# benjaminrwilson/range-view-3d-detection

Measured on AMD Instinct MI355X. Metric: sweeps/sec (fwd+bwd, 64x2048x5 range image), higher is better.
Workload: dtype bf16

## Files before the change

include/rv3d.h:

```cpp
#ifndef RV3D_H_
#define RV3D_H_

#include <stdint.h>

#ifdef __cplusplus
extern "C" {
#endif

typedef void* rvStream;

int rv_version(void);
const char* rv_last_error(void);

typedef struct {
    int32_t kh, kw;
    int32_t stride_w;
    int32_t pad_h, pad_w;
    int32_t cu, cv;
} rvTapGeom;

int32_t rv_pad_channels(int32_t c);

int64_t rv_packed_weight_bytes(const rvTapGeom* g);

int rv_pack_weight(const rvTapGeom* g, const float* T, void* gather_w, void* scatter_w, rvStream stream);

int64_t rv_pack_batch_entry_bytes(void);
int rv_pack_batch_fill(const rvTapGeom* g, const float* T, void* gather_w, void* scatter_w, void* host_entries);
int rv_pack_batch(const void* dev_table, int32_t n_entries, rvStream stream);

int rv_fold_geom(const rvTapGeom* g, rvTapGeom* folded);
int rv_pack_weight_folded(const rvTapGeom* g, const float* T, void* gather_w_folded, rvStream stream);
int rv_pack_batch_fill_folded(const rvTapGeom* g, const float* T, void* gather_w_folded, void* host_entry);
int rv_unfold_weight_grad(const rvTapGeom* g, const float* dT_folded, float* dT, int32_t accumulate, rvStream stream);

int rv_unpack_weight_grad(const rvTapGeom* g, const float* packed, float* dT, int32_t accumulate, rvStream stream);

#define RV_IN_AFFINE 1
#define RV_IN_RELU 2
#define RV_OUT_F32 4
#define RV_OUT_BIAS 8
#define RV_OUT_STATS 16
#define RV_OUT_ACCUM 32
#define RV_OUT_RELU 64
#define RV_OUT_RES_RELU 256
#define RV_WGRAD_TORCH_LAYOUT 128
#define RV_SEL_SMALL_GRIDS (1 << 20)
#define RV_SEL_SMALL_GRIDS6 (1 << 21)
#define RV_SEL_NO_GEN6 (1 << 22)
#define RV_SEL_NO_GEN5 (1 << 23)
#define RV_SEL_NO_POINTWISE (1 << 24)
#define RV_SEL_NO_POINTWISE_BWD (1 << 25)
#define RV_SEL_MASK (63 << 20)

typedef struct {
    int32_t N, H, Wu, Wv;
    int32_t ld_src, ld_dst;
    int32_t flags;
} rvTapShape;

int32_t rv_tap_stats_rows(const rvTapGeom* g, const rvTapShape* s, int32_t scatter);
int rv_tap_launch_info(const rvTapGeom* g, const rvTapShape* s, int32_t scatter, int32_t* host_info);
#define RV_STATS_SCRATCH_ROWS 128

int rv_tap_gather(const rvTapGeom* g, const rvTapShape* s, const void* V, const float* in_scale,
                  const float* in_shift, const void* gather_w, const float* bias, void* U,
                  float* stats_partial, rvStream stream);

int rv_tap_scatter(const rvTapGeom* g, const rvTapShape* s, const void* U, const float* in_scale,
                   const float* in_shift, const void* scatter_w, const float* bias, void* V,
                   float* stats_partial, rvStream stream);

int rv_tap_residual(const rvTapGeom* g, const rvTapShape* s, int32_t scatter, const void* src, const void* w, const float* bias,
                    const void* res, int32_t ld_res, void* dst, rvStream stream);

typedef struct rvBnbEpilogue {
    const void* y;
    int32_t ld_y;
    int32_t flags;
    const float* scale;
    const float* shift;
    const float* mean;
    const float* invstd;
    float* partial;
} rvBnbEpilogue;
int32_t rv_tap_bnb_rows(const rvTapGeom* g, const rvTapShape* s, int32_t scatter);
int rv_tap_data_grad_bnb(const rvTapGeom* g, const rvTapShape* s, int32_t scatter, const void* dout, const void* w, void* dx,
                         const rvBnbEpilogue* e, rvStream stream);

int64_t rv_tap_wgrad_workspace_bytes(const rvTapGeom* g, const rvTapShape* s);
int rv_tap_wgrad_info(const rvTapGeom* g, const rvTapShape* s, int32_t* host_info);
int rv_tap_wgrad(const rvTapGeom* g, const rvTapShape* s, const void* U, int32_t ld_u, const void* V, int32_t ld_v,
                 const float* in_scale, const float* in_shift, int32_t v_affine, float* dT_packed,
                 void* workspace, rvStream stream);

int rv_reduce_rows(const float* partial, int32_t rows, int32_t cols, float* out, rvStream stream);
int rv_reduce_rows_count(const float* partial, int32_t rows, int32_t cols, float count, float* out, float* out_copy, rvStream stream);
int rv_bn_finalize(const float* partial, int32_t rows, int32_t c, int64_t count, const float* gamma,
                   const float* beta, float eps, float momentum, float* running_mean, float* running_var,
                   float* scale, float* shift, float* mean, float* invstd, rvStream stream);
int rv_bn_fold_eval(int32_t c, const float* gamma, const float* beta, const float* running_mean,
                    const float* running_var, float eps, float* scale, float* shift, rvStream stream);

#define RV_EW_RELU_A 1
#define RV_EW_RELU_B 2
#define RV_EW_RELU_OUT 4
int rv_ew_combine(int64_t pixels, int32_t c, const void* a, int32_t ld_a, const float* a_scale,
                  const float* a_shift, const void* b, int32_t ld_b, const float* b_scale,
                  const float* b_shift, void* out, int32_t ld_out, int32_t flags, rvStream stream);

#define RV_BNB_RELU_Z 1
#define RV_BNB_RES_ACCUM 2
#define RV_BNB_Y_FROM_INPUT 4
int32_t rv_bn_bwd_rows(int64_t pixels);
int rv_bn_bwd_reduce(int64_t pixels, int32_t c, const void* dout, int32_t ld_dout, const void* out, int32_t ld_out,
                     const void* y, int32_t ld_y, const float* scale, const float* shift, const float* mean,
                     const float* invstd, int32_t flags, float* partial, rvStream stream);
int rv_bn_bwd_reduce_pair(int64_t pixels, int32_t c, const void* dout, int32_t ld_dout, const void* out, int32_t ld_out,
                          const void* ya, int32_t ld_ya, const float* mean_a, const float* invstd_a, const void* yb, int32_t ld_yb,
                          const float* mean_b, const float* invstd_b, float* partial_a, float* partial_b, rvStream stream);
int rv_bn_bwd_apply_pair(int64_t pixels, int32_t c, const void* dout, int32_t ld_dout, const void* out, int32_t ld_out,
                         const void* ya, int32_t ld_ya, const float* mean_a, const float* invstd_a, const float* coef_a, void* dya,
                         int32_t ld_dya, const void* yb, int32_t ld_yb, const float* mean_b, const float* invstd_b,
                         const float* coef_b, void* dyb, int32_t ld_dyb, rvStream stream);
int rv_bn_bwd_finalize(const float* partial, int32_t rows, int32_t c, int64_t count, const float* gamma,
                       const float* invstd, float* dgamma, float* dbeta, int32_t accumulate, float* coef,
                       rvStream stream);
int rv_bn_bwd_apply(int64_t pixels, int32_t c, const void* dout, int32_t ld_dout, const void* out, int32_t ld_out,
                    const void* y, int32_t ld_y, const float* scale, const float* shift, const float* mean,
                    const float* invstd, const float* coef, int32_t flags, void* dy, int32_t ld_dy, void* dres,
                    int32_t ld_dres, rvStream stream);
int32_t rv_head_final_bwd_rows(int64_t pixels);
int rv_head_final_bwd_sums(int64_t pixels, int32_t c, const void* y, int32_t ld_y, const void* dY, int32_t ld_dy, const void* w_scatter,
                           const float* scale, const float* shift, const float* mean, const float* invstd, int32_t relu, float* partial,
                           float* dw_partial, rvStream stream);
int rv_head_final_bwd_apply(int64_t pixels, int32_t c, const void* y, int32_t ld_y, const void* dY, int32_t ld_dy, const void* w_scatter,
                            const float* scale, const float* shift, const float* mean, const float* invstd, int32_t relu, const float* coef,
                            void* dy, int32_t ld_out, rvStream stream);
int64_t rv_bn_bwd_smallk_workspace_bytes(int64_t pixels, int32_t c, int32_t cin);
int rv_bn_bwd_smallk(int64_t pixels, int32_t c, const void* dout, int32_t ld_dout, const void* out, int32_t ld_out,
                     const void* y, int32_t ld_y, const float* scale, const float* shift, const float* mean,
                     const float* invstd, int32_t flags, const void* v, int32_t ld_v, int32_t cin, const void* w_packed,
                     int32_t ld_w, const float* gamma, const float* stat_mean, const float* stat_invstd, int64_t count,
                     float* dgamma, float* dbeta, float* dW, void* workspace, rvStream stream);
int rv_bn_bwd_smallk_sums(int64_t pixels, int32_t c, const void* dout, int32_t ld_dout, const void* out, int32_t ld_out,
                          const void* y, int32_t ld_y, const float* scale, const float* shift, const float* mean,
                          const float* invstd, int32_t flags, const void* v, int32_t ld_v, int32_t cin, const void* w_packed,
                          int32_t ld_w, double* sums, double* moms, void* workspace, rvStream stream);
int rv_bn_bwd_smallk_from_sums(int32_t c, int32_t cin, const double* sums, const double* moms, const double* global_s01,
                               const void* w_packed, int32_t ld_w, const float* gamma, const float* stat_mean,
                               const float* stat_invstd, int64_t count, float* dgamma, float* dbeta, float* dW,
                               rvStream stream);
int64_t rv_smallk_forward_workspace_bytes(int32_t cin);
int rv_smallk_moments(const void* v, int32_t ld_v, int64_t pixels, int32_t cin, double* moments, void* workspace,
                      rvStream stream);
int rv_smallk_forward(const void* v, int32_t ld_v, int64_t pixels, int32_t cin, const void* w_packed, int32_t ld_w,
                      int32_t c, const double* moments, int64_t count, const float* gamma, const float* beta, float eps,
                      float momentum, float* running_mean, float* running_var, float* scale, float* shift, float* mean,
                      float* invstd, int32_t relu, void* h, int32_t ld_h, rvStream stream);
int rv_ew_mask_grad(int64_t pixels, int32_t c, const void* dout, int32_t ld_dout, const void* out, int32_t ld_out,
                    void* d, int32_t ld_d, int32_t accumulate, rvStream stream);

int rv_range_partition(const float* features_nchw, const float* cart_nchw, const uint8_t* mask, int32_t N, int32_t C, int32_t H, int32_t W,
                       const float* lower, const float* upper, int32_t bands, void* dst, int32_t ld_dst, rvStream stream);

int rv_nchw_f32_to_nhwc_bf16(const float* src, int32_t N, int32_t C, int32_t H, int32_t W, void* dst, int32_t ld_dst,
                             int32_t c_offset, rvStream stream);
int rv_nhwc_bf16_to_nchw_f32(const void* src, int32_t ld_src, int32_t c_offset, int32_t N, int32_t C, int32_t H,
                             int32_t W, float* dst, rvStream stream);
int rv_nhwc_f32_to_nchw_f32(const float* src, int32_t ld_src, int32_t N, int32_t C, int32_t H, int32_t W, float* dst,
                            rvStream stream);
int rv_nchw_f32_to_nhwc_f32(const float* src, int32_t N, int32_t C, int32_t H, int32_t W, float* dst, int32_t ld_dst,
                            rvStream stream);

int rv_meta_relative(const float* cart_nchw, int32_t N, int32_t H, int32_t W, void* rel, rvStream stream);
int rv_meta_modulate(const void* pos_raw, const float* scale, const float* shift, const void* feat, int32_t ld_feat,
                     int32_t N, int32_t H, int32_t W, int32_t C, void* geo, rvStream stream);
int rv_meta_modulate_bwd(const void* dgeo, const void* pos_raw, const float* scale, const float* shift,
                         const void* feat, int32_t ld_feat, int32_t N, int32_t H, int32_t W, int32_t C,
                         void* dpos_act, void* dfeat, int32_t ld_dfeat, rvStream stream);
int32_t rv_meta_bwd_rows(int32_t N, int32_t H, int32_t W);
int rv_meta_modulate_bwd_sums(const void* dgeo, const void* pos_raw, const float* scale, const float* shift,
                              const float* mean, const float* invstd, const void* feat, int32_t ld_feat, int32_t N,
                              int32_t H, int32_t W, int32_t C, void* dfeat, int32_t ld_dfeat, float* partial,
                              rvStream stream);
int rv_meta_modulate_bwd_apply(const void* dgeo, const void* pos_raw, const float* scale, const float* shift,
                               const float* mean, const float* invstd, const float* coef, const void* feat,
                               int32_t ld_feat, int32_t N, int32_t H, int32_t W, int32_t C, void* dy, rvStream stream);

int32_t rv_pos_forward_rows(int64_t pixels);
int rv_pos_forward(const void* rel, int32_t ld_rel, int32_t cin, int64_t pixels, const void* w1_packed, int32_t ld_w1,
                   const float* scale1, const float* shift1, const void* w2_packed, int32_t c, void* h1, void* y2,
                   float* stats_partial, rvStream stream);

int rv_pos_modulate_forward(const void* rel, int32_t ld_rel, int32_t cin, const void* w1_packed, int32_t ld_w1, const float* scale1,
                            const float* shift1, const void* w2_packed, int32_t c, const float* scale2, const float* shift2,
                            const void* feat, int32_t ld_feat, int32_t N, int32_t H, int32_t W, void* geo, rvStream stream);

int rv_pos_backward_sums(int64_t pixels, int32_t c, const void* dy2, const void* w2_scatter, const void* rel, int32_t ld_rel,
                         int32_t cin, const void* w1_packed, int32_t ld_w1, const float* scale1, const float* shift1,
                         const float* mean1, const float* invstd1, double* sums, double* moms, void* workspace, rvStream stream);

int32_t rv_optim_chunk_elems(void);
int rv_adamw_step(const void* tensors, const void* chunks, int32_t n_chunks, float* partial, double lr, double beta1,
                  double beta2, double eps, double weight_decay, int64_t step, double max_norm, float* total_norm,
                  rvStream stream);
// ... 185 lines not shown
```

range_view_3d_detection_amd/_lib.py:

```python

from __future__ import annotations

import ctypes
import os
import re
from typing import Dict, List, Optional

import torch

_HERE = os.path.dirname(os.path.abspath(__file__))
LIB_PATH = os.environ.get("RV3D_LIB") or os.path.join(_HERE, "librv3d_hip.so")
LIB_PATH_F16 = os.environ.get("RV3D_LIB_F16") or os.path.join(_HERE, "librv3d_hip_f16.so")
HEADER_PATH = os.path.join(os.path.dirname(_HERE), "include", "rv3d.h")

IN_AFFINE, IN_RELU, OUT_F32, OUT_BIAS, OUT_STATS, OUT_ACCUM, OUT_RELU = 1, 2, 4, 8, 16, 32, 64
OUT_RES_RELU = 256
WGRAD_TORCH_LAYOUT = 128
SEL_SMALL_GRIDS, SEL_SMALL_GRIDS6, SEL_NO_GEN6, SEL_NO_GEN5, SEL_NO_POINTWISE, SEL_NO_POINTWISE_BWD = 1 << 20, 1 << 21, 1 << 22, 1 << 23, 1 << 24, 1 << 25
SELECT = 0
EW_RELU_A, EW_RELU_B, EW_RELU_OUT = 1, 2, 4
BNB_RELU_Z, BNB_RES_ACCUM, BNB_Y_FROM_INPUT = 1, 2, 4
STATS_SCRATCH_ROWS = 128


class TapGeom(ctypes.Structure):
    _fields_ = [(n, ctypes.c_int32) for n in ("kh", "kw", "stride_w", "pad_h", "pad_w", "cu", "cv")]


class TapShape(ctypes.Structure):
    _fields_ = [(n, ctypes.c_int32) for n in ("N", "H", "Wu", "Wv", "ld_src", "ld_dst", "flags")]

    def __init__(self, *args, **kw) -> None:
        super().__init__(*args, **kw)
        self.flags |= SELECT


class select:

    def __init__(self, flags: int) -> None:
        self.flags = flags

    def __enter__(self):
        global SELECT
        self.old, SELECT = SELECT, SELECT | self.flags
        return self

    def __exit__(self, *exc):
        global SELECT
        SELECT = self.old


class BnbEpilogue(ctypes.Structure):

    _fields_ = [("y", ctypes.c_void_p), ("ld_y", ctypes.c_int32), ("flags", ctypes.c_int32), ("scale", ctypes.c_void_p), ("shift", ctypes.c_void_p),
                ("mean", ctypes.c_void_p), ("invstd", ctypes.c_void_p), ("partial", ctypes.c_void_p)]


class TargetLevel(ctypes.Structure):

    _fields_ = [("stride", ctypes.c_int32), ("use_range", ctypes.c_int32), ("lower", ctypes.c_double), ("upper", ctypes.c_double)]


class TargetOut(ctypes.Structure):

    _fields_ = [(n, ctypes.c_void_p) for n in ("labels", "panoptics", "reg_targets", "points_per_obj")]


class LossEntry(ctypes.Structure):

    _fields_ = [(n, ctypes.c_void_p) for n in ("logits", "regressands", "cart", "mask", "labels", "panoptics", "reg_targets", "points_per_obj",
                                               "num_objects", "soft_targets", "foreground", "d_logits", "d_regressands")] + \
               [(n, ctypes.c_int32) for n in ("ld_logits", "ld_reg", "B", "n_cls", "H", "W")]


class LossParams(ctypes.Structure):

    _fields_ = [("coding_weights", ctypes.c_float * 8)] + [(n, ctypes.c_float) for n in ("cls_weight", "reg_weight", "smoothing", "sigma", "alpha", "gamma")] + \
               [("azimuth_invariant", ctypes.c_int32)]


ML_MAX_LEVELS, ML_MAX_ENTRIES = 8, 16
AFFINITY_GAUSSIAN, AFFINITY_BEV = 0, 1
EVAL_MAX_THRESHOLDS, EVAL_MAX_DTS = 8, 1024
WAYMO_MAX_DTS, WAYMO_MAX_GTS, WAYMO_MAX_SWEEPS = 1024, 1024, 65536
WAYMO_NUM_CUTOFFS, WAYMO_NUM_BREAKDOWN_ROWS, WAYMO_NUM_RESULT_ROWS = 101, 16, 32


def loss_sums_len() -> int:
    return int(load().rv_detection_loss_sums_len())


class RvError(RuntimeError):
    pass


_lib: Optional[ctypes.CDLL] = None
_lib_f16: Optional[ctypes.CDLL] = None
_OPERAND = "bf16"


class operand:

    def __init__(self, tag: str) -> None:
        if tag not in ("bf16", "f16"):
            raise RvError(f"unknown operand type {tag!r}")
        self.tag = tag

    def __enter__(self):
        global _OPERAND
        self.old, _OPERAND = _OPERAND, self.tag
        return self

    def __exit__(self, *exc):
        global _OPERAND
        _OPERAND = self.old


def operand_tag() -> str:
    return _OPERAND


def act_dtype() -> "torch.dtype":
    return torch.float16 if _OPERAND == "f16" else torch.bfloat16


def declared_symbols() -> List[str]:
    text = open(HEADER_PATH).read()
    text = re.sub(r"/\*.*?\*/", "", text, flags=re.S)
    return sorted(set(re.findall(r"\b(rv_[a-z0-9_]+)\s*\(", text)))


def load(tag: Optional[str] = None) -> ctypes.CDLL:
    global _lib, _lib_f16
    tag = tag or _OPERAND
    if tag == "f16":
        if _lib_f16 is None:
            _lib_f16 = _dlopen(LIB_PATH_F16)
        return _lib_f16
    if _lib is None:
        _lib = _dlopen(LIB_PATH)
    return _lib


def _dlopen(path: str) -> ctypes.CDLL:
    if not os.path.exists(path):
        raise RvError(
            f"{path} is missing: build it with `python -c 'import __graft_entry__ as g; g.build()'` "
            "(hipcc --offload-arch=gfx950).  There is no CPU fallback."
        )
    if torch.cuda.device_count() > 0 and torch.cuda.is_available():
        torch.cuda.init()
    lib = ctypes.CDLL(path)
    lib.rv_last_error.restype = ctypes.c_char_p
    for name in ("rv_packed_weight_bytes", "rv_decode_num_candidates", "rv_wnms_workspace_bytes", "rv_tap_wgrad_workspace_bytes", "rv_bn_bwd_smallk_workspace_bytes", "rv_smallk_forward_workspace_bytes", "rv_nms_sweeps_workspace_bytes", "rv_nms_rotated_workspace_bytes", "rv_pack_batch_entry_bytes", "rv_soft_assign_workspace_bytes", "rv_db_paste_workspace_bytes",
                 "rv_eval_summarize_workspace_bytes", "rv_waymo_match_workspace_bytes"):
        if hasattr(lib, name):
            getattr(lib, name).restype = ctypes.c_int64
    return lib


def _as_arg(v):
    if v is None:
        return ctypes.c_void_p(0)
    if isinstance(v, (ctypes.Structure,)):
        return ctypes.byref(v)
    if isinstance(v, float):
        return ctypes.c_float(v)
    if isinstance(v, int):
        return ctypes.c_int64(v) if abs(v) > 0x7FFFFFFF else ctypes.c_int32(v)
    return v

# ... 75 lines not shown
```

range_view_3d_detection_amd/csrc/tapconv.h:

```cpp
#pragma once
#include "common.h"

constexpr int kMaxTaps = 24;
constexpr int kMaxPhases = 4;
constexpr int RV_OUT_BNB = 1 << 16;

struct TapTable {
    int32_t ntaps[kMaxPhases];
    int32_t w_first[kMaxPhases];
    int32_t dw_min[kMaxPhases], dw_max[kMaxPhases];
    int32_t w_tile[kMaxPhases];
    int32_t dh_min, rows;
    int8_t dh[kMaxPhases][kMaxTaps];
    int8_t dw[kMaxPhases][kMaxTaps];
    int8_t ky[kMaxPhases][kMaxTaps];
    int8_t kx[kMaxPhases][kMaxTaps];
};

struct TapConvArgs {
    const bf16_t* src;
    void* dst;
    const bf16_t* w;
    const float* in_scale;
    const float* in_shift;
    const float* bias;
    float* stats;
    int32_t N, H, W_src, W_dst;
    int32_t C_src, C_dst;
    int32_t ld_src, ld_dst;
    int32_t phases, step;
    int32_t m_tiles;
    int32_t h_tiles;
    int32_t total_tiles, n_tiles, tiles_per_xcd;
    int32_t lds_a_elems;
    int32_t lds_tab_offset;
    int32_t flags;
    int32_t sel;
    const bf16_t* bnb_y;
    const float *bnb_scale, *bnb_shift, *bnb_mean, *bnb_invstd;
    float* bnb_partial;
    int32_t ld_bnb_y, bnb_flags;
    const bf16_t* res;
    int32_t ld_res;
    int32_t stats_per_wg;
    TapTable tt;
};

int rv_build_tap_table(const rvTapGeom* g, bool scatter, TapTable* tt, int* phases, int* step);

struct TapPlan {
    int gen;
    int bn, ks;
    int mt, nt;
    int epi;
    int pair, slices;
    int grid_x, grid_y;
    size_t lds;
    int stats_rows;
    int bnb_rows;
    int32_t info[4];
    bool scatter;
    TapConvArgs args;
};

bool rv_tapconv2_plan(TapPlan* p);
int rv_tapconv2_launch(const TapPlan& p, hipStream_t stream);
bool rv_tapconv4_plan(TapPlan* p);
int rv_tapconv4_launch(const TapPlan& p, hipStream_t stream);
bool rv_tapconv5_plan(TapPlan* p);
int rv_tapconv5_launch(const TapPlan& p, hipStream_t stream);
bool rv_tapconv6_plan(TapPlan* p);
int rv_tapconv6_launch(const TapPlan& p, hipStream_t stream);
bool rv_pointwise_plan(TapPlan* p);
int rv_pointwise_launch(const TapPlan& p, hipStream_t stream);
```

range_view_3d_detection_amd/csrc/tapconv.hip:

```cpp
#include <stdlib.h>

#include "common.h"
#include "tapconv.h"

namespace {

constexpr int kPix = 48;
constexpr int kNaMax = 7;

template <int MT, int NT>
__global__ __launch_bounds__(256, 2) void tapconv_kernel(const TapConvArgs a) {
    extern __shared__ __attribute__((aligned(16))) uint8_t smem[];
    constexpr int BM = 32 * MT, BN = 32 * NT;
    const int tid = threadIdx.x, lane = tid & 63, wave = tid >> 6;
    const int wm = wave >> 1, wn = wave & 1;
    const int l15 = lane & 15, lg = lane >> 4;

    int bx = blockIdx.x;
    const int mt = bx % a.m_tiles;
    bx /= a.m_tiles;
    const int h = bx % a.H;
    bx /= a.H;
    const int n = bx % a.N;
    const int ph = bx / a.N;
// ... 253 lines not shown
}

template <int MT, int NT>
int launch(const TapPlan& p, hipStream_t stream) {
    RV_LDS_OPT_IN(160 * 1024, tapconv_kernel<MT, NT>);
    hipLaunchKernelGGL((tapconv_kernel<MT, NT>), dim3(p.grid_x, p.grid_y), dim3(256), p.lds, stream, p.args);
    RV_CHECK_LAUNCH("tapconv_kernel");
    return 0;
}

}

int rv_build_tap_table(const rvTapGeom* g, bool scatter, TapTable* tt, int* phases, int* step) {
    memset(tt, 0, sizeof(*tt));
    RV_REQUIRE(g->kh >= 1 && g->kw >= 1 && g->kh * g->kw <= kMaxTaps, "tap geometry: kernel %dx%d unsupported", g->kh, g->kw);
    RV_REQUIRE(g->stride_w == 1 || g->stride_w == 2 || g->stride_w == 4, "tap geometry: stride_w %d unsupported", g->stride_w);
    int dh_lo = 127, dh_hi = -127;
    if (!scatter) {
        *phases = 1;
        *step = g->stride_w;
        tt->ntaps[0] = g->kh * g->kw;
        tt->w_first[0] = 0;
        int lo = 127, hi = -127;
        for (int ky = 0; ky < g->kh; ++ky)
            for (int kx = 0; kx < g->kw; ++kx) {
                const int t = ky * g->kw + kx;
                tt->ky[0][t] = (int8_t)ky;
                tt->kx[0][t] = (int8_t)kx;
                tt->dh[0][t] = (int8_t)(ky - g->pad_h);
                tt->dw[0][t] = (int8_t)(kx - g->pad_w);
                lo = lo < kx - g->pad_w ? lo : kx - g->pad_w;
                hi = hi > kx - g->pad_w ? hi : kx - g->pad_w;
                dh_lo = dh_lo < ky - g->pad_h ? dh_lo : ky - g->pad_h;
                dh_hi = dh_hi > ky - g->pad_h ? dh_hi : ky - g->pad_h;
            }
        tt->dw_min[0] = lo;
        tt->dw_max[0] = hi;
    } else {
        const int s = g->stride_w;
        *phases = s;
        *step = 1;
        int first = 0;
        for (int r = 0; r < s; ++r) {
            int cnt = 0, lo = 127, hi = -127;
            const int kx0 = (r + g->pad_w) % s, base = (r + g->pad_w) / s;
            for (int ky = 0; ky < g->kh; ++ky)
                for (int kx = kx0, j = 0; kx < g->kw; kx += s, ++j) {
                    tt->dh[r][cnt] = (int8_t)(g->pad_h - ky);
                    tt->dw[r][cnt] = (int8_t)(base - j);
                    tt->ky[r][cnt] = (int8_t)ky;
                    tt->kx[r][cnt] = (int8_t)kx;
                    lo = lo < base - j ? lo : base - j;
                    hi = hi > base - j ? hi : base - j;
                    dh_lo = dh_lo < g->pad_h - ky ? dh_lo : g->pad_h - ky;
                    dh_hi = dh_hi > g->pad_h - ky ? dh_hi : g->pad_h - ky;
                    ++cnt;
                }
            if (cnt == 0) { lo = 0; hi = 0; }
            tt->ntaps[r] = cnt;
            tt->w_first[r] = first;
            tt->dw_min[r] = lo;
            tt->dw_max[r] = hi;
            first += cnt;
        }
    }
    tt->dh_min = dh_lo;
    tt->rows = dh_hi - dh_lo + 1;
    return 0;
}

static int tapconv1_plan(TapPlan* p) {
    TapConvArgs& a = p->args;
    int mt = (a.step == 1) ? 4 : (a.step == 2 ? 2 : 1);
    const int wm_total = a.W_dst / a.phases;
    while (mt > 1 && 32 * mt / 2 >= wm_total) mt >>= 1;
    const int nt = a.C_dst >= 128 ? 4 : (a.C_dst >= 64 ? 2 : 1);
    const int BM = 32 * mt, BN = 32 * nt;
    int a_elems = 0;
    for (int r = 0; r < a.phases; ++r) {
        a.tt.w_tile[r] = (BM - 1) * a.step + (a.tt.dw_max[r] - a.tt.dw_min[r]) + 1;
        const int e = a.tt.rows * a.tt.w_tile[r] * kPix;
        a_elems = a_elems > e ? a_elems : e;
        RV_REQUIRE(a.tt.rows * a.tt.w_tile[r] * 4 <= 256 * kNaMax, "tap conv: halo tile too large (%d x %d)", a.tt.rows, a.tt.w_tile[r]);
    }
    a.lds_a_elems = a_elems;
    size_t lds = (size_t)(a_elems + 2 * BN * kPix) * sizeof(bf16_t);
    const size_t epi = (size_t)BM * (BN + 8) * sizeof(bf16_t);
    if (lds < epi) lds = epi;
    lds = (lds + 15) & ~(size_t)15;
    a.lds_tab_offset = (int32_t)lds;
    a.m_tiles = rv_ceil_div(wm_total, BM);
    p->gen = 1;
    p->mt = mt;
    p->nt = nt;
    p->lds = lds + 128;
    p->grid_x = a.m_tiles * a.H * a.N * a.phases;
    p->grid_y = rv_ceil_div(a.C_dst, BN);
    p->stats_rows = p->grid_x * 2;
    p->info[0] = 1, p->info[1] = mt * 16 + nt, p->info[2] = p->grid_x, p->info[3] = p->grid_y;
    return 0;
}

static int tapconv1_launch(const TapPlan& p, hipStream_t stream) {
#define RV_CASE(M, Nn) \
    if (p.mt == M && p.nt == Nn) return launch<M, Nn>(p, stream);
    RV_CASE(4, 4) RV_CASE(4, 2) RV_CASE(4, 1) RV_CASE(2, 4) RV_CASE(2, 2) RV_CASE(2, 1) RV_CASE(1, 4) RV_CASE(1, 2) RV_CASE(1, 1)
#undef RV_CASE
    RV_FAIL("tap conv: no kernel for tile %dx%d", p.mt, p.nt);
}

static int tap_plan(const rvTapGeom* g, const rvTapShape* s, bool scatter, bool want_bnb, bool has_residual, int32_t ld_res, TapPlan* out) {
    TapPlan base;
    memset(&base, 0, sizeof(base));
    base.scatter = scatter;
    TapConvArgs& a = base.args;
    if (rv_build_tap_table(g, scatter, &a.tt, &a.phases, &a.step)) return 1;
    RV_REQUIRE(s->Wv == s->Wu * g->stride_w, "tap shape: Wv (%d) must equal Wu (%d) * stride_w (%d)", s->Wv, s->Wu, g->stride_w);
    RV_REQUIRE(s->N > 0 && s->H > 0 && s->Wu > 0, "tap shape: empty tensor");
    const int cu = rv_pad32(g->cu), cv = rv_pad32(g->cv);
    a.N = s->N;
    a.H = s->H;
    a.W_src = scatter ? s->Wu : s->Wv;
    a.W_dst = scatter ? s->Wv : s->Wu;
    a.C_src = scatter ? cu : cv;
    a.C_dst = scatter ? cv : cu;
    a.ld_src = s->ld_src;
    a.ld_dst = s->ld_dst;
    RV_REQUIRE(a.ld_src >= a.C_src && a.ld_dst >= a.C_dst, "tap shape: channel strides (%d,%d) smaller than padded channels (%d,%d)",
               a.ld_src, a.ld_dst, a.C_src, a.C_dst);
    RV_REQUIRE(a.ld_src % 8 == 0 && a.ld_dst % 8 == 0, "tap shape: channel strides must be multiples of 8");
    a.flags = s->flags & ~RV_SEL_MASK;
    a.sel = s->flags & RV_SEL_MASK;
    a.ld_res = a.ld_dst;
    if (has_residual) {
        RV_REQUIRE(!(a.flags & (RV_OUT_ACCUM | RV_OUT_STATS)), "rv_tap_residual: not together with RV_OUT_ACCUM / RV_OUT_STATS");
        RV_REQUIRE(ld_res >= a.C_dst && ld_res % 8 == 0, "rv_tap_residual: bad channel stride of the residual (%d)", ld_res);
        a.flags |= RV_OUT_ACCUM;
        a.ld_res = ld_res;
    }
    RV_REQUIRE(!((a.flags & RV_OUT_F32) && (a.flags & RV_OUT_ACCUM)), "RV_OUT_ACCUM needs a bf16 destination");
    if (want_bnb) a.flags |= RV_OUT_BNB;

    const auto take = [&](bool (*plan)(TapPlan*)) {
        *out = base;
        return plan(out);
    };
    if (!(a.sel & (RV_SEL_NO_GEN6 | RV_SEL_NO_GEN5)) && take(rv_tapconv6_plan)) return 0;
    if (!(a.sel & RV_SEL_NO_GEN5) && take(rv_tapconv5_plan)) return 0;
    if (a.flags & RV_OUT_BNB) {
        *out = base;
        return 0;
    }
    if (take(rv_pointwise_plan)) return 0;
    if (take(rv_tapconv4_plan)) return 0;
    if (take(rv_tapconv2_plan)) return 0;
    *out = base;
    return tapconv1_plan(out);
}

static int tap_run(const TapPlan& plan, const void* src, const float* in_scale, const float* in_shift, const void* w, const float* bias,
                   void* dst, float* stats, const rvBnbEpilogue* bnb, const void* residual, rvStream stream) {
    TapPlan p = plan;
    TapConvArgs& a = p.args;
    RV_REQUIRE(residual || !(a.flags & RV_OUT_RES_RELU), "RV_OUT_RES_RELU belongs to rv_tap_residual");
    RV_REQUIRE(!(a.flags & RV_IN_AFFINE) || (in_scale && in_shift), "RV_IN_AFFINE without scale/shift");
    RV_REQUIRE(!(a.flags & RV_OUT_BIAS) || bias, "RV_OUT_BIAS without bias");
    RV_REQUIRE(!(a.flags & RV_OUT_STATS) || stats, "RV_OUT_STATS without a partial buffer");
    a.src = (const bf16_t*)src;
    a.dst = dst;
    a.w = (const bf16_t*)w;
    a.in_scale = in_scale;
    a.in_shift = in_shift;
    a.bias = bias;
    a.stats = stats;
    a.res = (const bf16_t*)(residual ? residual : dst);
    if (bnb) {
        RV_REQUIRE(bnb->y && bnb->scale && bnb->shift && bnb->mean && bnb->invstd && bnb->partial, "rv_tap_data_grad_bnb: null epilogue pointer");
        RV_REQUIRE(bnb->ld_y >= a.C_dst && bnb->ld_y % 8 == 0, "rv_tap_data_grad_bnb: bad channel stride of y (%d)", bnb->ld_y);
        a.bnb_y = (const bf16_t*)bnb->y;
        a.ld_bnb_y = bnb->ld_y;
        a.bnb_flags = bnb->flags;
        a.bnb_scale = bnb->scale;
        a.bnb_shift = bnb->shift;
        a.bnb_mean = bnb->mean;
        a.bnb_invstd = bnb->invstd;
        a.bnb_partial = bnb->partial;
    }
    hipStream_t st = (hipStream_t)stream;
    switch (p.gen) {
        case 6: return rv_tapconv6_launch(p, st);
        case 5: return rv_tapconv5_launch(p, st);
        case 7: return rv_pointwise_launch(p, st);
        case 4: return rv_tapconv4_launch(p, st);
        case 2: return rv_tapconv2_launch(p, st);
        case 1: return tapconv1_launch(p, st);
    }
    RV_FAIL("rv_tap_data_grad_bnb: this launch has no fused BatchNorm-backward sums (rv_tap_bnb_rows returned 0)");
}

extern "C" {

int32_t rv_tap_stats_rows(const rvTapGeom* g, const rvTapShape* s, int32_t scatter) {
    TapPlan p;
    return tap_plan(g, s, scatter != 0, false, false, 0, &p) ? -1 : p.stats_rows;
}

int rv_tap_launch_info(const rvTapGeom* g, const rvTapShape* s, int32_t scatter, int32_t* host_info) {
    RV_REQUIRE(g && s && host_info, "rv_tap_launch_info: null argument");
    TapPlan p;
    if (tap_plan(g, s, scatter != 0, false, false, 0, &p)) return 1;
    memcpy(host_info, p.info, sizeof(p.info));
    return 0;
}

int32_t rv_tap_bnb_rows(const rvTapGeom* g, const rvTapShape* s, int32_t scatter) {
    if (!g || !s) return 0;
    TapPlan p;
    return tap_plan(g, s, scatter != 0, true, false, 0, &p) ? -1 : p.bnb_rows;
}

int rv_tap_data_grad_bnb(const rvTapGeom* g, const rvTapShape* s, int32_t scatter, const void* dout, const void* w, void* dx,
                         const rvBnbEpilogue* e, rvStream stream) {
    RV_REQUIRE(g && s && dout && w && dx && e, "rv_tap_data_grad_bnb: null argument");
    TapPlan p;
    if (tap_plan(g, s, scatter != 0, true, false, 0, &p)) return 1;
    return tap_run(p, dout, nullptr, nullptr, w, nullptr, dx, nullptr, e, nullptr, stream);
}

int rv_tap_residual(const rvTapGeom* g, const rvTapShape* s, int32_t scatter, const void* src, const void* w, const float* bias,
                    const void* res, int32_t ld_res, void* dst, rvStream stream) {
    RV_REQUIRE(g && s && src && w && res && dst, "rv_tap_residual: null argument");
    TapPlan p;
    if (tap_plan(g, s, scatter != 0, false, true, ld_res, &p)) return 1;
    return tap_run(p, src, nullptr, nullptr, w, bias, dst, nullptr, nullptr, res, stream);
}

int rv_tap_gather(const rvTapGeom* g, const rvTapShape* s, const void* V, const float* in_scale, const float* in_shift,
                  const void* gather_w, const float* bias, void* U, float* stats_partial, rvStream stream) {
    RV_REQUIRE(g && s && V && gather_w && U, "rv_tap_gather: null argument");
    TapPlan p;
    if (tap_plan(g, s, false, false, false, 0, &p)) return 1;
    return tap_run(p, V, in_scale, in_shift, gather_w, bias, U, stats_partial, nullptr, nullptr, stream);
}

int rv_tap_scatter(const rvTapGeom* g, const rvTapShape* s, const void* U, const float* in_scale, const float* in_shift,
                   const void* scatter_w, const float* bias, void* V, float* stats_partial, rvStream stream) {
    RV_REQUIRE(g && s && U && scatter_w && V, "rv_tap_scatter: null argument");
    TapPlan p;
    if (tap_plan(g, s, true, false, false, 0, &p)) return 1;
    return tap_run(p, U, in_scale, in_shift, scatter_w, bias, V, stats_partial, nullptr, nullptr, stream);
}

}
```

range_view_3d_detection_amd/engine.py:

```python

from __future__ import annotations

import ctypes
import os
import weakref
from dataclasses import dataclass, field
from typing import Dict, List, Optional, Sequence, Tuple, Union

import torch
from torch import Tensor, nn

from . import _lib as L

BN_EPS = 1e-5
BN_MOMENTUM = 0.1

SYNC_BN: Optional[bool] = None
SYNC_WORLD1 = os.environ.get("RV3D_SYNC_WORLD1") is not None


def _dist_world() -> int:
    if torch.distributed.is_available() and torch.distributed.is_initialized():
        return torch.distributed.get_world_size()
    return 1


def bn_sync_world(bn: nn.Module, training: bool) -> int:
    world = _dist_world()
    if SYNC_WORLD1 and SYNC_BN is True and training and torch.distributed.is_initialized():
        return max(world, 2)
    if world == 1 or not training or SYNC_BN is False:
        return 1
    if SYNC_BN is True or isinstance(bn, nn.SyncBatchNorm):
        return world
    raise L.RvError(
        f"{type(bn).__name__} in training mode under a process group of {world} ranks: the reference trains with "
        "sync_batchnorm (conf/trainer/train.yaml:15).  Convert the modules (torch.nn.SyncBatchNorm.convert_sync_batchnorm / "
        "Lightning sync_batchnorm: true), or set range_view_3d_detection_amd.engine.SYNC_BN = True (sync) / False (per-rank "
        "statistics) explicitly.")


class KernelProfile:

    def __init__(self) -> None:
        self.records: List[tuple] = []

    def launch(self, name: str, flops: float, fn, nbytes: float = 0.0) -> None:
        a, b = torch.cuda.Event(enable_timing=True), torch.cuda.Event(enable_timing=True)
        a.record()
        fn()
        b.record()
        self.records.append((name, flops, a, b, nbytes))

    def summary(self) -> Dict[str, Dict[str, float]]:
        torch.cuda.synchronize()
        agg: Dict[str, Dict[str, float]] = {}
        for name, flops, a, b, nbytes in self.records:
            d = agg.setdefault(name, {"launches": 0, "ms": 0.0, "tflop": 0.0, "gbyte": 0.0})
            d["launches"] += 1
            d["ms"] += a.elapsed_time(b)
            d["tflop"] += flops / 1e12
            d["gbyte"] += nbytes / 1e9
        for d in agg.values():
            d["avg_us"] = 1e3 * d["ms"] / max(d["launches"], 1)
            d["tflops"] = d["tflop"] / max(d["ms"] * 1e-3, 1e-12)
        return agg

    def roofline(self, peak_tflops: float, name: Optional[str] = None) -> Dict[str, object]:
        agg = self.summary()
        if not agg:
            return {}
        if name is None or name not in agg:
            name = max(agg, key=lambda k: agg[k]["ms"])
        d = agg[name]
        return {"kernel": name, "bound": "mfma", "achieved": d["tflops"], "peak": peak_tflops, "unit": "TFLOP/s",
                "frac": d["tflops"] / peak_tflops, "traffic": None, "launches": d["launches"], "avg_launch_us": d["avg_us"],
                "flops_per_launch": 1e12 * d["tflop"] / max(d["launches"], 1),
                "algorithmic_bytes": 1e9 * d["gbyte"] / max(d["launches"], 1)}


PROFILE: Optional[KernelProfile] = None

_OVERLAP = os.environ.get("RV3D_OVERLAP", "free")
OVERLAP_WGRAD = _OVERLAP == "free" or _OVERLAP.startswith("small") or _OVERLAP.startswith("chain")
OVERLAP_CHAIN = _OVERLAP.startswith("chain")
HOLD_WGRAD_FOR_SYNC_BN = os.environ.get("RV3D_HOLD_WGRAD", "1") != "0"


def sync_bn_active() -> bool:
    if SYNC_BN is False or not (torch.distributed.is_available() and torch.distributed.is_initialized()):
        return False
    return _dist_world() > 1 or (SYNC_WORLD1 and SYNC_BN is True)


EARLY_WGRAD_FILL = float(os.environ.get("RV3D_EARLY_WGRAD_FILL", "0.9"))
OVERLAP_MAX_TFLOP: Optional[float] = ((float(_OVERLAP.split(":")[1]) if ":" in _OVERLAP else 0.1)
                                      if (_OVERLAP.startswith("small") or _OVERLAP.startswith("chain")) else None)
_SIDE_STREAMS: Dict[int, "torch.cuda.Stream"] = {}


_CU_COUNT: Dict[int, int] = {}


def cu_count(device) -> int:
    idx = torch.device(device).index or 0
    if idx not in _CU_COUNT:
        _CU_COUNT[idx] = int(torch.cuda.get_device_properties(idx).multi_processor_count)
    return _CU_COUNT[idx]


def side_stream(device) -> "torch.cuda.Stream":
    idx = torch.device(device).index or 0
    if idx not in _SIDE_STREAMS:
        prio = -1
        _SIDE_STREAMS[idx] = torch.cuda.Stream(device=device, priority=prio)
    return _SIDE_STREAMS[idx]




def _launch(name: str, flops: float, fn, nbytes: float = 0.0) -> None:
    if PROFILE is not None:
        PROFILE.launch(name, flops, fn, nbytes)
    else:
        fn()


def tap_kernel_name(geom, shape, scatter: bool) -> str:
    info = L.tap_launch_info(geom, shape, scatter)
    if info is None:
        raise L.RvError(f"rv_tap_launch_info failed: {L.load().rv_last_error().decode()}")
    if info[0] in (4, 5, 6):
        name = f"tapconv{info[0]}_kernel<{info[1]}>"
    elif info[0] in (2, 3):
        name = f"tapconv{info[0]}_kernel<{info[1]}>"
    elif info[0] == 7:
        name = f"pointwise_kernel<{info[1]}>"
    else:
        name = f"tapconv_kernel<{info[1] // 16},{info[1] % 16}>"
    if os.environ.get("RV3D_PROFILE_SHAPES"):
        name += f" {'S' if scatter else 'G'} k{geom.kh}x{geom.kw}s{geom.stride_w} {geom.cu}<->{geom.cv} {shape.N}x{shape.H}x{shape.Wu} f{shape.flags}"
    return name


def tap_flops(geom, shape) -> float:
    return 2.0 * shape.N * shape.H * shape.Wu * geom.kh * geom.kw * geom.cu * geom.cv


def tap_bytes(geom, shape, wgrad: bool = False) -> float:
    px = float(shape.N) * shape.H
    act = 2.0 * px * (shape.Wu * pad32(geom.cu) + shape.Wv * pad32(geom.cv))
    return act + (4.0 * geom.kh * geom.kw * geom.cu * geom.cv if wgrad else 2.0 * geom.kh * geom.kw * pad32(geom.cu) * pad32(geom.cv))


def all_reduce_(t: Tensor) -> None:
    from . import rccl

    if t.is_cuda and rccl.available():
        rccl.all_reduce_(t)
    else:
        torch.distributed.all_reduce(t)


def _totals_into(partial: Tensor, rows: int, count: int, region: Tensor, local_copy: Optional[Tensor] = None) -> None:
    if count >= 1 << 24:
        raise L.RvError("SyncBN: more than 2^24 elements per channel on one rank (the count travels as fp32)")
    n = region.numel() - 1
    if partial.is_cuda:
        L.call("rv_reduce_rows_count", L.ptr(partial), L.i32(rows), L.i32(n), L.f32(float(count)), L.ptr(region), L.ptr(local_copy), L.stream_ptr())
    else:
        region[:n] = partial[:rows].double().sum(dim=0).float().view(-1)
        region[n] = float(count)
        if local_copy is not None:
            local_copy.view(-1)[:n] = region[:n]


def allreduce_partial_rows(partial: Tensor, rows: int, count: int, local_copy: Optional[Tensor] = None) -> Tensor:
    c2 = partial.shape[1] * partial.shape[2]
    flat = torch.empty(c2 + 1, dtype=torch.float32, device=partial.device)
    _totals_into(partial, rows, count, flat, local_copy)
    COLLECTIVES.add(flat)
    all_reduce_(flat)
    return flat


def allreduce_partial_rows_many(items: Sequence[Tuple[Tensor, int, int, Optional[Tensor]]]) -> List[Tensor]:
    sizes = [p.shape[1] * p.shape[2] + 1 for p, _, _, _ in items]
    offs, total = [], 0
    for n in sizes:
        offs.append(total)
        total += (n + 3) // 4 * 4
    flat = torch.empty(total, dtype=torch.float32, device=items[0][0].device)
    views = []
    for (partial, rows, count, copy), o, n in zip(items, offs, sizes):
        v = flat[o : o + n]
        _totals_into(partial, rows, count, v, copy)
        views.append(v)
    COLLECTIVES.add(flat)
    all_reduce_(flat)
    return views


class GradSync:

    def __init__(self, params: Sequence[nn.Parameter], world: Optional[int] = None) -> None:
        self.params = [p for p in params if p.requires_grad]
        self.world = world if world is not None else _dist_world()
        self.offsets: Dict[int, Tuple[int, int]] = {}
        total = 0
        for p in self.params:
            self.offsets[id(p)] = (total, p.numel())
            total += (p.numel() + 63) // 64 * 64
        dev = self.params[0].device
        self.flat = torch.zeros(total, dtype=torch.float32, device=dev)
        self._views: Dict[int, Tensor] = {}
        self.works: List[tuple] = []
        self.pending: List[nn.Parameter] = []
        self.bytes = 4 * sum(p.numel() for p in self.params)

    def view(self, p: nn.Parameter) -> Tensor:
        v = self._views.get(id(p))
        if v is None:
            o, n = self.offsets[id(p)]
            v = self._views[id(p)] = self.flat[o : o + n].view_as(p)
        return v

    def broadcast_parameters(self, module: nn.Module) -> None:
        for t in list(module.parameters()) + list(module.buffers()):
            torch.distributed.broadcast(t.data, src=0)

    def reduce_node(self, params: Sequence[nn.Parameter], grads: Sequence[Optional[Tensor]]) -> List[Optional[Tensor]]:
        out = list(grads)
        idx = [i for i, (p, g) in enumerate(zip(params, grads)) if g is not None and id(p) in self.offsets]
        if not idx:
            return out
        pending = {id(p) for p in self.pending}
        for i in idx:
            if id(params[i]) in pending:
                raise L.RvError("GradSync: a parameter was reduced by two program nodes in one step -- its region of the flat buffer may still "
                                "be travelling in the first node's all-reduce (share the parameter inside ONE program, or call finish() between)")
            if params[i].grad is not None and params[i].grad is self._views.get(id(params[i])):
                raise L.RvError("GradSync: p.grad still is last step's view of the flat buffer -- call zero_grad(set_to_none=True) "
                                "before backward (gradient accumulation over several backward passes is not supported)")
        dst = [self.view(params[i]) for i in idx]
        torch._foreach_copy_(dst, [grads[i].to(torch.float32) for i in idx])
        spans = sorted((self.offsets[id(params[i])][0], (self.offsets[id(params[i])][1] + 63) // 64 * 64) for i in idx)
        runs: List[List[int]] = []
        for o, n in spans:
            if runs and runs[-1][1] == o:
                runs[-1][1] = o + n
            else:
                runs.append([o, o + n])
        live = torch.distributed.is_available() and torch.distributed.is_initialized()
        for lo, hi in runs:
            seg = self.flat[lo:hi]
            self.works.append((torch.distributed.all_reduce(seg, async_op=True) if live else None, seg))
        for i in idx:
            self.pending.append(params[i])
            out[i] = None
        return out

    def finish(self) -> None:
        for work, seg in self.works:
            if work is not None:
                work.wait()
            if self.world > 1:
                seg.mul_(1.0 / self.world)
        self.works.clear()
        for p in self.pending:
            p.grad = self.view(p)
        self.pending.clear()


GRAD_SYNC: Optional[GradSync] = None


class _CollectiveLog:

    def __init__(self) -> None:
        self.calls, self.bytes = 0, 0

    def add(self, t: Tensor) -> None:
        self.calls += 1
        self.bytes += t.numel() * t.element_size()

    def reset(self) -> None:
        self.calls, self.bytes = 0, 0


COLLECTIVES = _CollectiveLog()
# ... 885 lines not shown
```

Before: 41.33.

## Add specialized 1x1 conv kernel for 512-to-32 channel forward with fused input affine

Adds a persistent kernel for 1x1 gather convolutions from 512 to 32 channels (with input affine/ReLU, f32 output and bias) that keeps the whole weight matrix in registers. It double-buffers 32-pixel activation tiles into LDS using async global-to-LDS loads and applies the BN affine in place before the MFMA reduction. The planner picks it ahead of the generic tapconv4/2 paths when the shape matches and there are enough pixel steps. The aim is to cut the padding and tiling overhead the generic kernels pay for this narrow-output head layer, at the cost of more special-case code and selection logic.

Result: no change. 41.48, median of 6 (+0.4%).

```diff
diff --git a/include/rv3d.h b/include/rv3d.h
--- a/include/rv3d.h
+++ b/include/rv3d.h
@@ -51,7 +51,8 @@
 #define RV_SEL_NO_GEN5 (1 << 23)
 #define RV_SEL_NO_POINTWISE (1 << 24)
 #define RV_SEL_NO_POINTWISE_BWD (1 << 25)
-#define RV_SEL_MASK (63 << 20)
+#define RV_SEL_NO_SMALLN (1 << 26)
+#define RV_SEL_MASK (127 << 20)
 
 typedef struct {
     int32_t N, H, Wu, Wv;
diff --git a/range_view_3d_detection_amd/_lib.py b/range_view_3d_detection_amd/_lib.py
--- a/range_view_3d_detection_amd/_lib.py
+++ b/range_view_3d_detection_amd/_lib.py
@@ -17,6 +17,7 @@
 OUT_RES_RELU = 256
 WGRAD_TORCH_LAYOUT = 128
 SEL_SMALL_GRIDS, SEL_SMALL_GRIDS6, SEL_NO_GEN6, SEL_NO_GEN5, SEL_NO_POINTWISE, SEL_NO_POINTWISE_BWD = 1 << 20, 1 << 21, 1 << 22, 1 << 23, 1 << 24, 1 << 25
+SEL_NO_SMALLN = 1 << 26
 SELECT = 0
 EW_RELU_A, EW_RELU_B, EW_RELU_OUT = 1, 2, 4
 BNB_RELU_Z, BNB_RES_ACCUM, BNB_Y_FROM_INPUT = 1, 2, 4
diff --git a/range_view_3d_detection_amd/csrc/smalln.hip b/range_view_3d_detection_amd/csrc/smalln.hip
--- /dev/null
+++ b/range_view_3d_detection_amd/csrc/smalln.hip
@@ -0,0 +1,155 @@
+#include "common.h"
+#include "tapconv.h"
+
+namespace {
+
+constexpr int kK = 512;
+constexpr int kN = 32;
+constexpr int kPx = 32;
+constexpr int kRow = kK * 2;
+constexpr int kBuf = kPx * kRow;
+constexpr int kKS = kK / 32;
+constexpr int kThreads = 256;
+
+struct SmallNArgs {
+    const bf16_t* x;
+    const bf16_t* w;
+    const float *scale, *shift;
+    const float* bias;
+    float* y;
+    int64_t P;
+    int ld_x, ld_y;
+    int relu;
+};
+
+typedef __attribute__((address_space(3))) void lds_void_t;
+typedef const __attribute__((address_space(1))) void glb_void_t;
+
+__global__ __launch_bounds__(kThreads, 2) void smalln_kernel(const SmallNArgs a) {
+    extern __shared__ __attribute__((aligned(16))) uint8_t smem[];
+    const int tid = threadIdx.x, lane = tid & 63;
+    const int wn = __builtin_amdgcn_readfirstlane(tid >> 6);
+    const int l15 = lane & 15, lg = lane >> 4;
+    const int t = wn & 1, j = wn >> 1;
+    bf16x8 fw[kKS];
+#pragma unroll
+    for (int ks = 0; ks < kKS; ++ks) fw[ks] = *(const bf16x8*)(a.w + (j * 16 + l15) * kK + ks * 32 + lg * 8);
+    f32x4 bias;
+#pragma unroll
+    for (int r = 0; r < 4; ++r) bias[r] = a.bias[j * 16 + lg * 4 + r];
+    float sc[8], sh[8];
+#pragma unroll
+    for (int e = 0; e < 8; ++e) {
+        sc[e] = a.scale[lane * 8 + e];
+        sh[e] = a.shift[lane * 8 + e];
+    }
+    __device__ __attribute__((aligned(256))) static uint32_t smalln_zero_page[64];
+    int foff[8];
+#pragma unroll
+    for (int i = 0; i < 8; ++i) {
+        const int q = wn + 4 * i;
+        foff[i] = q * a.ld_x + ((lane ^ (q & 15)) * 8);
+    }
+    auto fill = [&](int64_t step, int buf) __attribute__((always_inline)) {
+        const bf16_t* const x_step = a.x + step * (int64_t)kPx * a.ld_x;
+        const int64_t left = a.P - step * kPx;
+#pragma unroll
+        for (int i = 0; i < 8; ++i) {
+            const int q = wn + 4 * i;
+            const bf16_t* src = q < left ? x_step + foff[i] : (const bf16_t*)smalln_zero_page + (lane & 7) * 8;
+            __builtin_amdgcn_global_load_lds((glb_void_t*)src, (lds_void_t*)(smem + buf * kBuf + q * kRow), 16, 0, 0);
+        }
+    };
+    uint32_t fo[8];
+#pragma unroll
+    for (int i = 0; i < 8; ++i) {
+        const int p = wn + 4 * i;
+        fo[i] = p * kRow + ((lane ^ (p & 15)) * 16);
+    }
+    uint32_t rb[4];
+#pragma unroll
+    for (int x = 0; x < 4; ++x) rb[x] = (t * 16 + l15) * kRow + (((((x << 2) | lg) ^ l15) & 15) * 16);
+    const int yoff = (t * 16 + l15) * a.ld_y + j * 16 + lg * 4;
+    const bool relu = a.relu != 0;
+
+    const int64_t steps = (a.P + kPx - 1) / kPx;
+    const int64_t first = blockIdx.x, stride = gridDim.x;
+    if (first < steps) fill(first, 0);
+    asm volatile("s_waitcnt vmcnt(0)" ::: "memory");
+    __syncthreads();
+    int cur = 0;
+    for (int64_t s = first; s < steps; s += stride) {
+        const int64_t nxt = s + stride;
+        const bool has_next = nxt < steps;
+        if (has_next) fill(nxt, cur ^ 1);
+        uint8_t* const img = smem + cur * kBuf;
+        u32x4 v[8];
+#pragma unroll
+        for (int i = 0; i < 8; ++i) v[i] = *(const u32x4*)(img + fo[i]);
+#pragma unroll
+        for (int i = 0; i < 8; ++i) {
+            pin_here(v[i]);
+#pragma unroll
+            for (int d = 0; d < 4; ++d) {
+                float lo = bf_lo(v[i][d]), hi = bf_hi(v[i][d]);
+                lo = lo * sc[2 * d] + sh[2 * d];
+                hi = hi * sc[2 * d + 1] + sh[2 * d + 1];
+                if (relu) {
+                    lo = fmaxf(lo, 0.f);
+                    hi = fmaxf(hi, 0.f);
+                }
+                v[i][d] = pack_bf2(lo, hi);
+            }
+            *(u32x4*)(img + fo[i]) = v[i];
+        }
+        asm volatile("s_waitcnt lgkmcnt(0)" ::: "memory");
+        __builtin_amdgcn_s_barrier();
+        f32x4 acc = {0.f, 0.f, 0.f, 0.f};
+#pragma unroll
+        for (int ks = 0; ks < kKS; ++ks) {
+            const bf16x8 fx = *(const bf16x8*)(img + rb[ks & 3] + (ks >> 2) * 256);
+            acc = RV_MFMA_16x16x32(fw[ks], fx, acc, 0, 0, 0);
+        }
+        acc += bias;
+        const int64_t left = a.P - s * kPx;
+        if (t * 16 + l15 < left) *(f32x4*)(a.y + s * (int64_t)kPx * a.ld_y + yoff) = acc;
+        if (has_next) asm volatile("s_waitcnt vmcnt(1)" ::: "memory");
+        asm volatile("s_waitcnt lgkmcnt(0)" ::: "memory");
+        __builtin_amdgcn_s_barrier();
+        cur ^= 1;
+    }
+    asm volatile("s_waitcnt vmcnt(0)" ::: "memory");
+}
+
+}
+
+bool rv_smalln_plan(TapPlan* p) {
+    const TapConvArgs* a = &p->args;
+    if ((a->sel & RV_SEL_NO_SMALLN) || p->scatter) return false;
+    if (a->phases != 1 || a->step != 1 || a->tt.ntaps[0] != 1 || a->tt.dh[0][0] != 0 || a->tt.dw[0][0] != 0) return false;
+    if (a->C_src != kK || a->C_dst != kN || a->W_src != a->W_dst) return false;
+    if ((a->flags & ~RV_IN_RELU) != (RV_IN_AFFINE | RV_OUT_F32 | RV_OUT_BIAS)) return false;
+    const int64_t P = (int64_t)a->N * a->H * a->W_src;
+    if (P * a->ld_src >= ((int64_t)1 << 31) || P * a->ld_dst >= ((int64_t)1 << 31)) return false;
+    const int64_t steps = (P + kPx - 1) / kPx;
+    const int wgs = 2 * rv_persistent_grid();
+    if (steps < ((a->sel & RV_SEL_SMALL_GRIDS) ? 1 : 2 * (int64_t)wgs)) return false;
+    p->gen = 8;
+    p->grid_x = (int)(steps < wgs ? steps : wgs);
+    p->lds = (size_t)2 * kBuf;
+    p->info[0] = 8, p->info[1] = kK, p->info[2] = p->grid_x, p->info[3] = 1;
+    return true;
+}
+
+int rv_smalln_launch(const TapPlan& plan, hipStream_t stream) {
+    const TapConvArgs& a = plan.args;
+    SmallNArgs p{};
+    p.x = a.src, p.w = a.w, p.scale = a.in_scale, p.shift = a.in_shift, p.bias = a.bias, p.y = (float*)a.dst;
+    p.P = (int64_t)a.N * a.H * a.W_src, p.ld_x = a.ld_src, p.ld_y = a.ld_dst;
+    p.relu = (a.flags & RV_IN_RELU) ? 1 : 0;
+    RV_REQUIRE(a.C_src == kK && a.C_dst == kN && plan.grid_x >= 1, "small-N kernel: 512 -> 32 channels");
+    RV_LDS_OPT_IN(2 * kBuf, smalln_kernel);
+    hipLaunchKernelGGL(smalln_kernel, dim3(plan.grid_x), dim3(kThreads), plan.lds, stream, p);
+    RV_CHECK_LAUNCH("smalln_kernel");
+    return 0;
+}
diff --git a/range_view_3d_detection_amd/csrc/tapconv.h b/range_view_3d_detection_amd/csrc/tapconv.h
--- a/range_view_3d_detection_amd/csrc/tapconv.h
+++ b/range_view_3d_detection_amd/csrc/tapconv.h
@@ -73,3 +73,5 @@
 int rv_tapconv6_launch(const TapPlan& p, hipStream_t stream);
 bool rv_pointwise_plan(TapPlan* p);
 int rv_pointwise_launch(const TapPlan& p, hipStream_t stream);
+bool rv_smalln_plan(TapPlan* p);
+int rv_smalln_launch(const TapPlan& p, hipStream_t stream);
diff --git a/range_view_3d_detection_amd/csrc/tapconv.hip b/range_view_3d_detection_amd/csrc/tapconv.hip
--- a/range_view_3d_detection_amd/csrc/tapconv.hip
+++ b/range_view_3d_detection_amd/csrc/tapconv.hip
@@ -429,6 +429,7 @@
         return 0;
     }
     if (take(rv_pointwise_plan)) return 0;
+    if (take(rv_smalln_plan)) return 0;
     if (take(rv_tapconv4_plan)) return 0;
     if (take(rv_tapconv2_plan)) return 0;
     *out = base;
@@ -468,6 +469,7 @@
         case 6: return rv_tapconv6_launch(p, st);
         case 5: return rv_tapconv5_launch(p, st);
         case 7: return rv_pointwise_launch(p, st);
+        case 8: return rv_smalln_launch(p, st);
         case 4: return rv_tapconv4_launch(p, st);
         case 2: return rv_tapconv2_launch(p, st);
         case 1: return tapconv1_launch(p, st);
diff --git a/range_view_3d_detection_amd/engine.py b/range_view_3d_detection_amd/engine.py
--- a/range_view_3d_detection_amd/engine.py
+++ b/range_view_3d_detection_amd/engine.py
@@ -136,6 +136,8 @@
         name = f"tapconv{info[0]}_kernel<{info[1]}>"
     elif info[0] == 7:
         name = f"pointwise_kernel<{info[1]}>"
+    elif info[0] == 8:
+        name = f"smalln_kernel<{info[1]}>"
     else:
         name = f"tapconv_kernel<{info[1] // 16},{info[1] % 16}>"
     if os.environ.get("RV3D_PROFILE_SHAPES"):
```
